# peterdavidfagan/mujoco_robot_environments

Measured on AMD Instinct MI355X. Metric: env steps/sec (whole node), RearrangementEnv batch=4096 at 1/2/4/8 MI355X, higher is better.
Workload: dtype f32

## Files before the change

### mujoco_robot_environments_amd/csrc/mre_dev.h

```cpp
#pragma once
#include <stdint.h>

namespace mre {

constexpr int NB = 20;
constexpr int NRB = 16;
constexpr int GRIP_BODY0 = 8;
constexpr int NV = 39;
constexpr int NRV = 15;
constexpr int NQ = 43;
constexpr int NQP = 44;
constexpr int TRACE_W = 88;
constexpr int TRACE_QVEL = 48;
constexpr int NVP = 40;
constexpr int NU = 8;
constexpr int QFINE = 32;
constexpr int QFINE_ROW = 96;
constexpr int QFINE_CUBE_Q = 32;
constexpr int QFINE_CUBE_V = 60;
static_assert(QFINE_CUBE_Q + 7 * 4 == QFINE_CUBE_V && QFINE_CUBE_V + 6 * 4 <= QFINE_ROW, "qfine row layout");
constexpr int NPROP = 4;
constexpr int NG = 20;
constexpr int PROP_GEOM0 = 12;
constexpr int NPAIR = 128;
// ... 156 lines not shown

struct StepArgs {
  const DevModel* M;
  int N;
  float* qpos;
  float* qvel;
  float* qacc_ws;
  float* qfine;
  float* ctrl;
  const float* ctrl_seq;
  int seq_stride;
  const int* nprops;
  const float* prop_size;
  int nsteps, control_steps, mode;
  unsigned flags;
  const OscConfig* osc;
  int osc_stride;
  const float* osc_target;
  const uint8_t* grip_closed;
  uint8_t* converged;
  float* sites;
  uint32_t* status;
  int* nstep;
  int* stats;
  float* trace;
  int trace_nenv, trace_max, trace_base;
  const uint8_t* env_mask;
  const int* env_order;
  float* geoms;
  float* contacts;
  float* contacts_full;
  int* settle_steps;
  int min_settle_steps;
  const uint8_t* large;
  int want_large;
  float *sv_qpos, *sv_qvel, *sv_qacc_ws, *sv_qfine, *sv_ctrl;
  int* sv_nstep;
  uint32_t* sv_status;
  uint8_t* sv_converged;
  int* launch_info;
  uint8_t* pending;
  int* q_head;
  int* q_tail;
  int* q_buf;
  int* q_acc;
  int* q_done;
  int* q_started;
  const int* q_gen;
  int q_gen_expect;
  int q_wait;
  int* q_err;
  int q_nticks, q_shards, q_cap, q_stride;
  int q_lshards, q_capl;
};
constexpr int QUEUE_TICKS_MAX = 256;
constexpr int QUEUE_SHARDS_MAX = 32;
constexpr int QUEUE_LSHARDS_MAX = 16;

struct SearchArgs {
  const DevModel* M;
  int N;
  float* qpos;
  const int* nprops;
  const float* prop_size;
  const uint8_t* env_mask;
  const long long* env_ids;
  long long env_id_offset;
  unsigned long long seed;
  const int* prop;
  int fixed_prop;
  const double* bounds;
  double shared_bounds[6];
  const int* tick_base;
  long long tick0;
  int max_attempts;
  int yaw_mode;
  double fixed_quat[4];
  float max_dist;
  int commit;
  float* qfine;
  double* pose;
  int* attempts;
  unsigned flags;
};

constexpr int DYN_W = 128;
constexpr int DYN_JAC = 0, DYN_MASS = 42, DYN_BIAS = 91, DYN_POS = 98, DYN_QUAT = 101, DYN_QPOS = 105, DYN_QVEL = 112,
              DYN_PAD = 119;
struct DynArgs {
  const DevModel* M;
  int N;
  const float* qpos;
  const float* qvel;
  const float* qfine;
  const int* nprops;
  const float* prop_size;
  int site;
  float* out;
};

struct SortArgs {
  const DevModel* M;
  int N;
  const float* qpos;
  const int* nprops;
  const double* zones;
// ... 30 lines not shown
```

### mujoco_robot_environments_amd/csrc/mre_env.h

```cpp
#pragma once
#include <hip/hip_runtime.h>

#include <string>
#include <utility>
#include <vector>

#include "../../include/mre.h"
#include "mre_dev.h"
#include "mre_policy.h"

#define HIPCHK(x)                                                                       \
  do {                                                                                  \
    hipError_t e_ = (x);                                                                \
    if (e_ != hipSuccess)                                                               \
      return mre::fail(MRE_ERR_HIP, std::string(#x) + ": " + hipGetErrorString(e_));    \
  } while (0)

struct mre_env {
  int N = 0, device = 0;
  hipStream_t stream = nullptr;
  mre::DevModel* dM = nullptr;
  mre::DevModel hM;
  int solver = MRE_SOLVER_PGS;
  float *qpos = nullptr, *qvel = nullptr, *qacc_ws = nullptr, *ctrl = nullptr;
// ... 29 lines not shown
  std::vector<std::pair<hipEvent_t, hipEvent_t>> events;
  size_t events_used = 0;
  bool fallback = true;
  unsigned base_flags = 0;
  bool large_only = false;
  bool compact_only = false;
  hipStream_t stream2 = nullptr;
  hipEvent_t ev_fork = nullptr, ev_join = nullptr, ev_order = nullptr;
  uint8_t *d_large = nullptr, *mask_r = nullptr;
  float *sv_qpos = nullptr, *sv_qvel = nullptr, *sv_qacc_ws = nullptr, *sv_ctrl = nullptr, *sv_qfine = nullptr;
  uint32_t* sv_status = nullptr;
  uint8_t* sv_converged = nullptr;
  float* contacts = nullptr;
  float* contacts_full = nullptr;
  int* settle_steps = nullptr;
  int* h_launch_info = nullptr;
  int* d_launch_info = nullptr;
  int* h_info_last = nullptr;
  uint8_t* d_pending = nullptr;
  uint8_t* h_large_stage = nullptr;
  uint8_t* d_large_stage = nullptr;
  bool d_large_stale = false;
  std::vector<uint8_t> h_large, h_rerun;
  int n_large = 0;
  long long* d_env_ids = nullptr;
  int *ps_attempts = nullptr, *ps_prop = nullptr, *ps_tick = nullptr, *ps_which = nullptr;
  double *ps_bounds = nullptr, *ps_pose = nullptr, *ps_zones = nullptr, *ps_pick = nullptr;
  int last_settle_max = 0;
  long long n_reruns = 0, n_promotions = 0, n_demotions = 0;
  struct Group {
    int lo = 0, n = 0;
    hipStream_t st = nullptr, st2 = nullptr;
    hipEvent_t ev_fork = nullptr, ev_join = nullptr;
    struct Out {
      mre::StepArgs args;
      hipEvent_t ev_info = nullptr;
      int stage = 0;
    } out[mre::policy::RING];
    int head = 0, nout = 0;
    int cur = 0;
    int* h_order = nullptr;
    int* d_order = nullptr;
  };
  std::vector<Group> groups;
  int* h_grp_order = nullptr;
  int* d_grp_order = nullptr;
  Group qgroup;
  bool queue_ok = true;
  int queue_ticks = 200;
  int queue_waves = 0;
  int queue_shards = 16;
  int queue_lshards = 8;
  bool queue_test_serial = false;
  int queue_spare_large = 8;
  int queue_run_ticks = 100;
  int queue_min_ticks = 32;
  float tick_tail = 0.f;
  bool tick_tail_valid = false;
  float queue_tail_min = 1.45f;
  unsigned tail_samples = 0;
  std::vector<int> tail_scratch;
  int queue_large_waves_max = 0;
  int* h_qlist = nullptr;
  int* q_ws = nullptr;
  int* q_gen = nullptr;
  int* h_q_err = nullptr;
  int* h_qgrp_order = nullptr;
  long n_queue_launches = 0;
  long long n_handovers = 0;
  int queue_last_handovers = 0;
  static constexpr int RING = mre::policy::RING;
  int ring = 2;
  static constexpr int NSTAGE = mre::policy::NSTAGE;
  hipEvent_t ev_main = nullptr;
  float* seq_copy[RING + 1] = {nullptr, nullptr, nullptr, nullptr, nullptr};
  size_t seq_cap = 0;
  unsigned seq_calls = 0;
  double dbg_wait_s = 0, dbg_call_s = 0; long dbg_calls = 0;
  int calls_since_drain = 0, sync_streak = 0;
  bool broken = false;
};

namespace mre {
int fail(int code, const std::string& msg);
int sched_create(mre_env* e);
void sched_destroy(mre_env* e);
int launch_step(mre_env* e, const StepArgs& a, bool settle = false, bool pipeline_ok = true, bool allow_queue = false);
int drain(mre_env* e, bool api_call = false);
}
#define DRAIN(e) do { int rc_ = mre::drain(e, true); if (rc_) return rc_; } while (0)
#define DRAIN_PENDING(e) do { int rc_ = mre::drain(e, false); if (rc_) return rc_; } while (0)

inline int profile_events(mre_env* e, hipEvent_t* e0, hipEvent_t* e1) {
  *e0 = *e1 = nullptr;
  if (!e->profiling) return MRE_OK;
  if (e->events_used == e->events.size()) {
    hipEvent_t x, y;
    HIPCHK(hipEventCreate(&x)); HIPCHK(hipEventCreate(&y));
    e->events.emplace_back(x, y);
  }
  *e0 = e->events[e->events_used].first; *e1 = e->events[e->events_used].second;
  e->events_used++;
  return MRE_OK;
}
```

### mujoco_robot_environments_amd/csrc/mre_kernels.hip

```cpp
#include <hip/hip_runtime.h>

#include "mre_dev.h"
#include "mre_math.h"
#include "mre_collide.h"

namespace mre {
using ModelP = MRE_MODEL_PTR(DevModel);
#if defined(MRE_PHASE_STAMPS) && MRE_PHASE_STAMPS >= 4
__shared__ unsigned long long dbg_acc[4];
#endif

struct OscSm {
  float J[6][7], M[7][7], MiJt[7][6], Li[6][6], Lam[6][6], V[6][6], Jbar[7][6];
  float ep[3], eo[3], F[6], LF[6], tn[7], Jbt[6], xd[6], w[6];
};

struct alignas(8) Blk {
  uint16_t row0;
  uint8_t type, nrows;
  uint8_t rslot;
  uint8_t pa, pb;
  uint8_t primary : 4;
  uint8_t bslot : 4;
};
// ... 1229 lines not shown
    return 1;
  }
}
MRE_DEV bool queue_pop(const StepArgs& a, int l, int home, int& env, int& tick, int& shard) {
  const int S = a.q_shards;
  if (Q_LARGE) {
    const int SL = a.q_lshards;
    for (unsigned idle = 0;; ++idle) {
      int r = 0;
      for (int k = 0; k < SL && r == 0; ++k) {
        const int sh = S + (home + k < SL ? home + k : home + k - SL);
        r = queue_pop_shard(a, l, sh, env, tick);
        if (r != 0) shard = sh;
      }
      if (r != 0) return r > 0;
      if (a.q_wait == 0 || q_load(a.q_done) >= a.N) return false;
      if (idle > 512u && q_load(a.q_started) == 0) return false;
      if (idle > (1u << 18)) return false;
      __builtin_amdgcn_s_sleep(127);
    }
  }
  for (int k = 0; k < S; ++k) {
    const int sh = home + k < S ? home + k : home + k - S;
    const int r = queue_pop_shard(a, l, sh, env, tick);
    if (r != 0) { shard = sh; return r > 0; }
  }
  return false;
}
MRE_DEV void queue_push(const StepArgs& a, int l, int env, int tick, int shard) {
  __builtin_amdgcn_fence(__ATOMIC_RELEASE, "agent");
  asm volatile("s_waitcnt vmcnt(0)" ::: "memory");
  if (l == 0) {
    const int i = __hip_atomic_fetch_add(a.q_tail + shard * QUEUE_TICKS_MAX + tick, 1, __ATOMIC_RELAXED, __HIP_MEMORY_SCOPE_AGENT);
    __hip_atomic_store(q_bucket(a, tick, shard) + i, env + 1, __ATOMIC_RELAXED, __HIP_MEMORY_SCOPE_AGENT);
  }
}

template <bool QUEUE>
MRE_DEV void step_body(const StepArgs& a, Sm& s) {
  OscSm& osc = s.osc;
  const int l = threadIdx.x;
  int env = 0, qtick = 0, qshard = 0;
  if (!QUEUE) {
    if ((int)blockIdx.x >= a.N) return;
    env = a.env_order != nullptr ? a.env_order[blockIdx.x] : (int)blockIdx.x;
  }
  if (QUEUE && !Q_LARGE && l == 0) __hip_atomic_fetch_add(a.q_started, 1, __ATOMIC_RELAXED, __HIP_MEMORY_SCOPE_AGENT);
  if (QUEUE && Q_LARGE && a.q_wait != 0) {
    for (unsigned idle = 0; q_load(a.q_gen) != a.q_gen_expect; ++idle) {
      if (idle > 1024u) return;
      __builtin_amdgcn_s_sleep(127);
    }
  }
 for (;;) {
  if (QUEUE) {
    if (!queue_pop(a, l, (int)(blockIdx.x % (unsigned)(Q_LARGE ? a.q_lshards : a.q_shards)), env, qtick, qshard)) return;
    if (qtick > 0 || Q_LARGE) __builtin_amdgcn_fence(__ATOMIC_ACQUIRE, "agent");
  }
  const int step_lo = QUEUE ? qtick * a.control_steps : 0, step_hi = QUEUE ? step_lo + a.control_steps : a.nsteps;
  if (QUEUE && !Q_LARGE && qtick == 0 && a.large != nullptr && a.large[env] != 0) continue;
  if (!QUEUE || (!Q_LARGE && qtick == 0)) {
#define MRE_PASS_SKIP { if (QUEUE) { if (l == 0) __hip_atomic_fetch_add(a.q_done, 1, __ATOMIC_RELAXED, __HIP_MEMORY_SCOPE_AGENT); continue; } return; }
  if (!QUEUE && a.large != nullptr && (a.large[env] != 0) != (a.want_large != 0)) return;
  if (a.env_mask != nullptr && a.env_mask[env] == 0) {
    if (a.launch_info != nullptr && l < 4) a.launch_info[(size_t)env * 4 + l] = -1;
    MRE_PASS_SKIP;
  }
  if (a.pending != nullptr && a.pending[env] != 0) {
    if (a.launch_info != nullptr && l < 4) a.launch_info[(size_t)env * 4 + l] = l == 0 ? -2 : -1;
    MRE_PASS_SKIP;
  }
#undef MRE_PASS_SKIP
  }
  ModelP M = (ModelP)a.M;

  const bool save = a.sv_qpos != nullptr && step_lo == 0;
  if (l < NQP) {
    const float v = a.qpos[(size_t)env * NQP + l];
    s.qpos[l] = v;
    if (save) a.sv_qpos[(size_t)env * NQP + l] = v;
  }
  if (l < NVP) {
    const float v = a.qvel[(size_t)env * NVP + l], w = a.qacc_ws[(size_t)env * NVP + l];
    s.qvel[l] = v;
    s.qacc[l] = w;
    s.qfrc_con[l] = 0.f;
    if (save) { a.sv_qvel[(size_t)env * NVP + l] = v; a.sv_qacc_ws[(size_t)env * NVP + l] = w; }
  }
  if (l < QFINE) {
    const float v = a.qfine != nullptr ? a.qfine[(size_t)env * QFINE_ROW + l] : 0.f;
    s.qlo[l] = v;
    if (save && a.qfine != nullptr) a.sv_qfine[(size_t)env * QFINE_ROW + l] = v;
  }
  if (save && a.qfine != nullptr && l < QFINE_ROW - QFINE)
    a.sv_qfine[(size_t)env * QFINE_ROW + QFINE + l] = a.qfine[(size_t)env * QFINE_ROW + QFINE + l];
  float cube_lo_keep = 0.f;
  if (QUEUE && !Q_LARGE && a.qfine != nullptr && l < QFINE_ROW - QFINE) cube_lo_keep = a.qfine[(size_t)env * QFINE_ROW + QFINE + l];
  if (l < NU) {
    const float v = a.ctrl[(size_t)env * NU + l];
    s.ctrl[l] = v;
    if (save) a.sv_ctrl[(size_t)env * NU + l] = v;
  }
  if (save && l == 0) {
    if (a.nstep != nullptr) a.sv_nstep[env] = a.nstep[env];
    a.sv_status[env] = a.status[env];
    a.sv_converged[env] = a.converged != nullptr ? a.converged[env] : (uint8_t)0;
  }
  if (l == 0) { s.nprops = a.nprops[env]; s.overflow = 0; s.ncon = 0; s.nefc = 0; s.solver_iters = 0; }
#ifdef MRE_NEWTON
  if (l < 24) s.zrow[l] = 0.f;
#endif
  if (l < NPROP * 3) {
    const float sz = a.prop_size[(size_t)env * NPROP * 3 + l];
    s.prop_size[l / 3][l % 3] = sz;
  }
  MRE_SYNC();
  if (l < NPROP) {
    const float m = M->body_mass[NRB + l];
    const float* z = s.prop_size[l];
    s.prop_mass[l] = m;
    s.prop_inertia[l][0] = m / 3.f * (z[1] * z[1] + z[2] * z[2]);
    s.prop_inertia[l][1] = m / 3.f * (z[0] * z[0] + z[2] * z[2]);
    s.prop_inertia[l][2] = m / 3.f * (z[0] * z[0] + z[1] * z[1]);
  }
  MRE_SYNC();

#if defined(MRE_PHASE_STAMPS) && MRE_PHASE_STAMPS >= 4
  if (l < 4) dbg_acc[l] = 0ull;
#endif
#ifdef MRE_PHASE_STAMPS
  unsigned long long stamp_acc[4] = {0, 0, 0, 0};
  unsigned long long stamp_t = __builtin_amdgcn_s_memtime();
#endif
  bool arm_converged = ((a.flags & F_CONV_CONTINUE) != 0 || (QUEUE && qtick > 0)) && a.converged != nullptr && a.converged[env] != 0;
  float grip_cmd = 0.f;
  const OscConfig* oscp = a.osc + (size_t)env * a.osc_stride;
  int hw_ncon = 0, hw_nefc = 0, hw_nrrow = 0, hw_npp = 0;
  const unsigned long long launch_t0 = __builtin_amdgcn_s_memtime();
  if (a.mode == CTRL_OSC) {
    if (l < 16) s.osc_tgt[l] = a.osc_target[(size_t)env * 16 + l];
    grip_cmd = a.grip_closed[env] ? M->act_ctrlrange[NU - 1][1] : M->act_ctrlrange[NU - 1][0];
    MRE_SYNC();
  }
  int steps_done = 0;
  bool settled = false;
  for (int step = step_lo; step < step_hi; ++step) {
    MRE_STAMP(7);
    position_stage(M, s, l);
    MRE_STAMP(12);
    MRE_STAMP(13);
    gripper_local(M, s, l);
    if ((a.flags & F_NO_CONSTRAINTS) == 0) connect_rows_local(M, s, l);
    MRE_STAMP(14);
    crb_mass_matrix(M, s, l);
    MRE_SYNC();
#ifndef MRE_NEWTON
    factor_robot_regs(s.qM, s.qLD, s.qLDinv);
#endif
    MRE_STAMP(15);
    MRE_STAMP(0);

    velocity_stage(M, s, l);
    MRE_SYNC();
    finger_bias(M, s, l);
    MRE_STAMP(1);
    const bool constrained = (a.flags & F_NO_CONSTRAINTS) == 0;
    if (constrained) {

      collide(M, s, l, false, (a.flags & F_CLIP_ALWAYS) != 0);
      MRE_STAMP(2);
      assemble_constraints(M, s, l);
#ifdef MRE_NEWTON
      nw_build_lists(s, l);
#else
      solve_robot_rows(s, l);
      assemble_blocks(M, s, l);
#endif
      MRE_STAMP(3);
      hw_ncon = max(hw_ncon, s.ncon); hw_nefc = max(hw_nefc, s.nefc);
      hw_nrrow = max(hw_nrrow, s.nrrow); hw_npp = max(hw_npp, s.npp);
    }

    if (a.mode == CTRL_SEQ && (step % a.control_steps) == 0) {
      const int tick = step / a.control_steps;
      if (l < NU) s.ctrl[l] = a.ctrl_seq[((size_t)tick * a.seq_stride + env) * NU + l];
      MRE_SYNC();
    }
    if (a.mode == CTRL_OSC && (step % a.control_steps) == 0) {
      if (step > 0 && osc_converged(M, s, oscp, s.osc_tgt)) arm_converged = true;
      osc_compute(M, s, osc, oscp, s.osc_tgt, l);
      if (l == 0) s.ctrl[NU - 1] = grip_cmd;
      MRE_SYNC();
// ... 88 lines not shown
    MRE_SYNC();
  }
  if (a.nsteps == 0 && (a.flags & F_DETECT) != 0 && a.contacts != nullptr) {
    position_stage(M, s, l);
    collide(M, s, l, (a.flags & F_DETECT_ACTIVE) == 0, (a.flags & F_CLIP_ALWAYS) != 0);
    float* o = a.contacts + (size_t)env * (1 + 3 * CONTACT_EXPORT);
    const int n = s.ncon < CONTACT_EXPORT ? s.ncon : CONTACT_EXPORT;
    if (l == 0) o[0] = s.overflow ? -(float)s.ncon : (float)s.ncon;
    if (l < n) {
      const int pr = s.con_pair[l];
      o[1 + 3 * l] = (float)M->pair_g1[pr]; o[2 + 3 * l] = (float)M->pair_g2[pr]; o[3 + 3 * l] = s.con_dist[l];
      if (a.contacts_full != nullptr) {
        float* f = a.contacts_full + ((size_t)env * CONTACT_EXPORT + l) * 12;
        for (int k = 0; k < 3; k++) f[k] = s.con_pos[l][k];
        for (int k = 0; k < 9; k++) f[3 + k] = s.con_frame[l][k];
      }
    }
    MRE_SYNC();
    if (l == 0) s.overflow = 0;
  }
  const bool q_last = !QUEUE || (qtick + 1 == a.q_nticks && !hand_over);
  if (q_last && (a.mode == CTRL_OSC || a.sites != nullptr || a.geoms != nullptr)) kinematics_only(M, s, l);
  if (a.mode == CTRL_OSC && a.nsteps > 0 && !hand_over) {
    if (q_last && osc_converged(M, s, oscp, s.osc_tgt)) arm_converged = true;
    if (l == 0) {
      if (a.converged != nullptr) a.converged[env] = arm_converged ? 1 : 0;
      if (q_last && !arm_converged && a.status != nullptr && (a.flags & F_CONV_OPEN) == 0) {
        if (QUEUE) __hip_atomic_fetch_or(a.status + env, 1u, __ATOMIC_RELAXED, __HIP_MEMORY_SCOPE_AGENT);
        else a.status[env] |= 1u;
      }
    }
  }
  if (a.geoms != nullptr && l < NG) {
    float p[3], R[9], size[3], rb;
    geom_pose(M, s, l, p, R, size, &rb);
    float* o = a.geoms + ((size_t)env * NG + l) * 16;
    const int pid = M->geom_propid[l];
    const bool active = pid < 0 || pid < s.nprops;
    for (int k = 0; k < 3; k++) o[k] = p[k];
    for (int k = 0; k < 9; k++) o[3 + k] = R[k];
    for (int k = 0; k < 3; k++) o[12 + k] = size[k];
    o[15] = active ? (float)M->geom_type[l] : -1.f;
  }
  if (a.sites != nullptr && q_last) {
    float* o = a.sites + (size_t)env * 16;
    if (l < 3) o[l] = s.site_xpos[M->opt_rec.tcp_site][l];
    if (l >= 3 && l < 6) o[l] = s.site_xpos[M->opt_rec.eef_site][l - 3];
    if (l == 6) {
      float q[4];
      mat2q(q, s.site_xmat[0]);
      o[6] = q[0]; o[7] = q[1]; o[8] = q[2]; o[9] = q[3];
    }
  }
  if (hand_over) {
    if (a.qfine != nullptr && l < QFINE_ROW - QFINE) a.qfine[(size_t)env * QFINE_ROW + QFINE + l] = cube_lo_keep;
  } else {
    if (l < NQP) a.qpos[(size_t)env * NQP + l] = s.qpos[l];
    if (l < NVP) {
      a.qvel[(size_t)env * NVP + l] = s.qvel[l];
      a.qacc_ws[(size_t)env * NVP + l] = l < NV ? s.qacc[l] : 0.f;
    }
    if (l < QFINE && a.qfine != nullptr) a.qfine[(size_t)env * QFINE_ROW + l] = s.qlo[l];
    if (l < NU) a.ctrl[(size_t)env * NU + l] = s.ctrl[l];
  }
  const bool q_more = QUEUE && !hand_over && qtick + 1 < a.q_nticks;
  if (l == 0 && a.launch_info != nullptr) {
    int* li = a.launch_info + (size_t)env * 4;
    unsigned long long dt = (__builtin_amdgcn_s_memtime() - launch_t0) >> 10;
    int moved = 0;
    if (QUEUE) {
      int* qa = a.q_acc + (size_t)env * 4;
      if (qtick > 0 || Q_LARGE) {
        hw_ncon = max(hw_ncon, q_load(qa + 0) & 0xFFFF); hw_nefc = max(hw_nefc, q_load(qa + 1));
        hw_nrrow = max(hw_nrrow, q_load(qa + 2) & 0xFFFF); hw_npp = max(hw_npp, q_load(qa + 2) >> 16);
        dt += (unsigned long long)q_load(qa + 3);
        moved = q_load(qa + 0) >> 16;
      }
      if (hand_over) moved = 1;
      if (q_more || hand_over) { qa[0] = hw_ncon | (moved << 16); qa[1] = hw_nefc; qa[2] = hw_nrrow | (hw_npp << 16); qa[3] = (int)dt; }
      else dt /= (unsigned long long)(qtick + 1);
    }
    if (!q_more && !hand_over) {
#ifdef MRE_LARGE_CAPS
      li[0] = (s.overflow ? 2 : 0) | (moved ? 4 : 0);
#else
      li[0] = s.overflow ? 1 : 0;
#endif
      li[1] = hw_ncon | ((int)(dt < 0x7FFFull ? dt : 0x7FFFull) << 16); li[2] = hw_nefc; li[3] = hw_nrrow | (hw_npp << 16);
    }
  }
#ifndef MRE_LARGE_CAPS
  if (!QUEUE && l == 0 && a.pending != nullptr && s.overflow) a.pending[env] = 1;
#endif
  if (l == 0 && a.status != nullptr && !hand_over) {
    unsigned st = 0;
    for (int k = 0; k < NQ; k++) if (!isfinite(s.qpos[k])) st |= 2u;
    if (s.overflow) st |= 4u;
    if (QUEUE) { if (st) __hip_atomic_fetch_or(a.status + env, st, __ATOMIC_RELAXED, __HIP_MEMORY_SCOPE_AGENT); }
    else a.status[env] |= st;
    if (a.stats != nullptr && a.nsteps > 0) {
      a.stats[env * 4 + 0] = s.ncon; a.stats[env * 4 + 1] = s.nefc;
      a.stats[env * 4 + 2] = s.solver_iters; a.stats[env * 4 + 3] = s.nl;
#ifdef MRE_PHASE_STAMPS
      for (int k = 0; k < 4; k++) a.stats[env * 4 + k] = (int)(stamp_acc[k] >> 4);
#if MRE_PHASE_STAMPS >= 4
      for (int k = 0; k < 4; k++) a.stats[env * 4 + k] = (int)(dbg_acc[k] >> 4);
#endif
#endif
    }
  }
  if (!QUEUE) return;
  if (hand_over) queue_push(a, l, env, qtick, a.q_shards + env % a.q_lshards);
  else if (q_more) queue_push(a, l, env, qtick + 1, qshard);
  else if (l == 0) __hip_atomic_fetch_add(a.q_done, 1, __ATOMIC_RELAXED, __HIP_MEMORY_SCOPE_AGENT);
 }
}

#ifdef MRE_NEWTON
#define MRE_VARIANT(name) name##_newton
#else
#define MRE_VARIANT(name) name
#endif

#ifdef MRE_LARGE_CAPS
__global__ __launch_bounds__(64, 2) void MRE_VARIANT(k_step_large)(StepArgs a) {
  __shared__ Sm s;
  step_body<false>(a, s);
}
}

extern "C" void MRE_VARIANT(mre_launch_step_large)(const mre::StepArgs* args, hipStream_t stream) {
  hipLaunchKernelGGL(mre::MRE_VARIANT(k_step_large), dim3(args->N), dim3(64), 0, stream, *args);
}
namespace mre {
__global__ __launch_bounds__(64, 2) void MRE_VARIANT(k_step_queue_large)(StepArgs a) {
  __shared__ Sm s;
  step_body<true>(a, s);
}
}
extern "C" void MRE_VARIANT(mre_launch_step_queue_large)(const mre::StepArgs* args, int nwaves, hipStream_t stream) {
  hipLaunchKernelGGL(mre::MRE_VARIANT(k_step_queue_large), dim3(nwaves), dim3(64), 0, stream, *args);
}
#else
__global__ __launch_bounds__(64, 2) void MRE_VARIANT(k_step)(StepArgs a) {
  __shared__ Sm s;
  step_body<false>(a, s);
}

__global__ __launch_bounds__(64, 2) void MRE_VARIANT(k_settle)(StepArgs a) {
  __shared__ Sm s;
  step_body<false>(a, s);
}

__global__ __launch_bounds__(64, 2) void MRE_VARIANT(k_step_queue)(StepArgs a) {
  __shared__ Sm s;
  step_body<true>(a, s);
}

#ifdef MRE_NEWTON
}
extern "C" void mre_launch_step_newton(const mre::StepArgs* args, hipStream_t stream) {
  hipLaunchKernelGGL(mre::k_step_newton, dim3(args->N), dim3(64), 0, stream, *args);
}
extern "C" void mre_launch_settle_newton(const mre::StepArgs* args, hipStream_t stream) {
  hipLaunchKernelGGL(mre::k_settle_newton, dim3(args->N), dim3(64), 0, stream, *args);
}
extern "C" void mre_launch_step_queue_newton(const mre::StepArgs* args, int nwaves, hipStream_t stream) {
// ... 346 lines not shown
```

### mujoco_robot_environments_amd/csrc/mre_policy.h

```cpp
#pragma once
#include <algorithm>

#include "mre_dev.h"

namespace mre {
namespace policy {

constexpr int RING = 4;
constexpr int NSTAGE = RING + 1;

inline int info_duration(const int* li) { return li[0] < 0 ? 0 : (li[1] >> 16); }

inline int compact_nrrow_max(bool newton) { return newton ? NRROW_MAX_COMPACT_NEWTON : NRROW_MAX_COMPACT_PGS; }
inline bool near_compact_caps(bool newton, int hw_ncon, int hw_nefc, int hw_nrrow, int hw_npp) {
  return 8 * hw_ncon > 7 * NCON_MAX || 8 * hw_nefc > 7 * NEFC_MAX || 8 * hw_nrrow > 7 * compact_nrrow_max(newton) || 8 * hw_npp > 7 * NPP_MAX;
}
inline bool far_below_compact_caps(bool newton, int hw_ncon, int hw_nefc, int hw_nrrow, int hw_npp) {
  return 8 * hw_ncon <= 5 * NCON_MAX && 8 * hw_nefc <= 5 * NEFC_MAX && 8 * hw_nrrow <= 5 * compact_nrrow_max(newton) && 8 * hw_npp <= 5 * NPP_MAX;
}

enum Action {
  NONE,
  RERUN,
  PROMOTE,
// ... 15 lines not shown
  for (int i = lo; i < lo + n; i++) kmax = std::max(kmax, info_duration(info + 4 * (size_t)i));
  if (kmax == 0) return 0;
  int count[258] = {0};
  auto bucket = [&](int i) { return (int)((long long)info_duration(info + 4 * (size_t)i) * 255 / kmax); };
  for (int i = lo; i < lo + n; i++) count[255 - bucket(i) + 1]++;
  for (int k = 1; k <= 256; k++) count[k] += count[k - 1];
  for (int i = lo; i < lo + n; i++) order[lo + count[255 - bucket(i)]++] = i;
  return kmax;
}

inline bool tick_tail_ratio(const int* info, int lo, int n, int* scratch, float* ratio) {
  size_t m = 0;
  long long sum = 0;
  for (int i = lo; i < lo + n; i++) {
    const int* li = info + 4 * (size_t)i;
    if (li[0] >= 0) { scratch[m++] = li[1] >> 16; sum += li[1] >> 16; }
  }
  if (m < 256 || sum <= 0) return false;
  const size_t k = m - 1 - m / 100;
  std::nth_element(scratch, scratch + k, scratch + m);
  *ratio = (float)scratch[k] * (float)m / (float)sum;
  return true;
}

inline int free_stage(int cur, const int* younger_stages, int nyounger) {
  bool used[NSTAGE] = {false};
  used[cur] = true;
  for (int k = 0; k < nyounger; k++) used[younger_stages[k]] = true;
  int fs = 0;
  while (used[fs]) fs++;
  return fs;
}

inline int queue_large_waves(const int* info_last, const uint8_t* large, int lo, int n, int nl, int last_handovers,
                             int spare_large, int large_waves_max ) {
  int lw = nl + std::max(last_handovers, spare_large);
  double wl = 0, wc = 0;
  for (int i = lo; i < lo + n; i++) {
    const double d = (double)info_duration(info_last + 4 * (size_t)i);
    if (large[i]) wl += d; else wc += d;
  }
  const double ncomp = (double)(n - nl);
  const double r = (wl > 0 && wc > 0) ? wl / wc : (ncomp > 0 ? 1.3 * (double)nl / ncomp : 1e9);
  const double x = r * 160.0 / (26.5 * r + 20.4);
  const int bal = std::max((int)(x * (double)(large_waves_max / 2)), large_waves_max / 4);
  return std::max(std::min(lw, bal), 1);
}

inline bool queue_fits(bool queue_ok, int queue_waves, int N) { return queue_ok && queue_waves > 0 && N > queue_waves; }
inline bool window_wants_queue(int nticks, int queue_min_ticks, bool tick_tail_valid, float tick_tail, float queue_tail_min) {
  return nticks >= queue_min_ticks || (nticks >= 8 && !(tick_tail_valid && tick_tail < queue_tail_min));
}

inline int ring_keep(int nsteps, int ring) { return nsteps <= 50 ? ring - 1 : 0; }

}
}
```

### mujoco_robot_environments_amd/csrc/mre_sched.cpp

```cpp
#include <hip/hip_runtime.h>
#include <chrono>
#include <cstdlib>
#include <cstring>

#include "mre_env.h"
#include "mre_launch.h"

using namespace mre;

static void launch_compact(const mre_env* e, const StepArgs& a, hipStream_t st, bool settle = false) {
  const StepKernels& K = step_kernels(e->solver);
  (settle ? K.settle : K.step)(&a, st);
}
static void launch_large(const mre_env* e, const StepArgs& a, hipStream_t st) { step_kernels(e->solver).large(&a, st); }

static int launch_split(const mre_env* e, const StepArgs& a, bool run_large, bool settle, hipStream_t st, hipStream_t st2,
                        hipEvent_t ev_fork, hipEvent_t ev_join) {
  StepArgs ac = a;
  ac.want_large = 0;
  if (run_large) {
    HIPCHK(hipEventRecord(ev_fork, st));
    HIPCHK(hipStreamWaitEvent(st2, ev_fork, 0));
    StepArgs al = a;
    al.want_large = 1;
// ... 105 lines not shown
  }
  bool any = e->qgroup.nout > 0;
  for (auto& G : e->groups) any = any || G.nout > 0;
  if (!any) return MRE_OK;
  HIPCHK(hipSetDevice(e->device));
  for (auto& G : e->groups) {
    int rc = drain_group(e, G, true);
    if (rc) return rc;
  }
  return drain_group(e, e->qgroup, true);
}

static void guard_args(mre_env* e, StepArgs& a) {
  a.large = e->d_large; a.launch_info = e->d_launch_info;
  a.sv_qpos = e->sv_qpos; a.sv_qvel = e->sv_qvel; a.sv_qacc_ws = e->sv_qacc_ws; a.sv_qfine = e->sv_qfine;
  a.sv_ctrl = e->sv_ctrl; a.sv_status = e->sv_status; a.sv_converged = e->sv_converged; a.sv_nstep = e->sv_nstep;
}

static int launch_group_enqueue(mre_env* e, mre_env::Group& G, const StepArgs& a_full, bool queue) {
  int rc;
  StepArgs a = a_full;
  const size_t N = (size_t)e->N;
  if (G.nout == 0) {
    memcpy(e->h_large_stage + (size_t)G.cur * N + G.lo, e->h_large.data() + G.lo, (size_t)G.n);
    (void)policy::sort_longest_first(e->h_info_last, G.lo, G.n, G.h_order + (size_t)G.cur * N);
  }
  a.N = G.n; a.env_order = G.d_order + (size_t)G.cur * N + G.lo; a.seq_stride = e->N;
  hipEvent_t p0, p1;
  rc = profile_events(e, &p0, &p1);
  if (rc) return rc;
  HIPCHK(hipStreamWaitEvent(G.st, e->ev_main, 0));
  if (p0) HIPCHK(hipEventRecord(p0, G.st));
  guard_args(e, a);
  a.pending = e->d_pending;
  const int slot = (G.head + G.nout) % mre_env::RING;
  a.large = e->d_large_stage + (size_t)G.cur * N;
  a.launch_info = e->d_launch_info + (size_t)slot * 4 * N;
  const uint8_t* const fl = e->h_large_stage + (size_t)G.cur * N;
  if (queue) {
    StepArgs ac = a;
    ac.want_large = 0;
    const StepKernels& K = step_kernels(e->solver);
    const int nt = a.nsteps / a.control_steps, S = e->queue_shards, cap = (G.n + S - 1) / S;
    const int SL = e->queue_lshards, capl = (G.n + SL - 1) / SL;
    constexpr int QS = QUEUE_SHARDS_MAX + QUEUE_LSHARDS_MAX;
    const size_t ctl = 2 * (size_t)QS * QUEUE_TICKS_MAX + 16;
    const size_t stride = (size_t)S * cap + (size_t)SL * capl;
    const size_t words = ctl + 4 * N + (size_t)nt * stride;
    ac.sv_qpos = nullptr;
    ac.q_head = e->q_ws; ac.q_tail = ac.q_head + QS * QUEUE_TICKS_MAX;
    ac.q_done = ac.q_tail + QS * QUEUE_TICKS_MAX; ac.q_started = ac.q_done + 1; ac.q_acc = ac.q_done + 16;
    ac.q_buf = ac.q_acc + 4 * N; ac.q_err = e->h_q_err; ac.q_nticks = nt; ac.q_shards = S; ac.q_cap = cap; ac.q_stride = (int)stride;
    ac.q_lshards = SL; ac.q_capl = capl;
    ac.q_gen = e->q_gen; ac.q_gen_expect = (int)(e->n_queue_launches + 1);
    int* const hl = e->h_qlist + (size_t)(e->n_queue_launches % (mre_env::RING + 1)) * (N + 32);
    int nl = 0;
    for (int j = 0; j < SL; j++) hl[j] = 0;
    memset(hl + 16, 0, (size_t)SL * capl * 4);
    for (int i = G.lo; i < G.lo + G.n; i++)
      if (fl[i]) { const int j = i % SL; hl[16 + (size_t)j * capl + hl[j]++] = i + 1; nl++; }
    StepArgs al = ac;
    al.want_large = 1; al.q_wait = 1;
    const int lw = policy::queue_large_waves(e->h_info_last, fl, G.lo, G.n, nl, e->queue_last_handovers, e->queue_spare_large,
                                             e->queue_large_waves_max);
    hipStream_t const st_large = e->queue_test_serial ? G.st : G.st2;
    K.queue_large(&al, lw, st_large);
    HIPCHK(hipGetLastError());
    HIPCHK(hipEventRecord(G.ev_join, st_large));
    HIPCHK(hipMemsetAsync(e->q_ws, 0, ((words * 4 + 15) / 16) * 16, G.st));
    if (nl > 0) {
      HIPCHK(hipMemcpyAsync(ac.q_buf + (size_t)S * cap, hl + 16, (size_t)SL * capl * 4, hipMemcpyHostToDevice, G.st));
      HIPCHK(hipMemcpy2DAsync(ac.q_tail + S * QUEUE_TICKS_MAX, (size_t)QUEUE_TICKS_MAX * 4, hl, 4, 4, (size_t)SL, hipMemcpyHostToDevice, G.st));
    }
    HIPCHK(hipMemsetD32Async((hipDeviceptr_t)e->q_gen, ac.q_gen_expect, 1, G.st));
    const int nwaves = G.n < e->queue_waves ? G.n : e->queue_waves;
    K.queue(&ac, nwaves, G.st);
    HIPCHK(hipGetLastError());
    al.q_wait = 0;
    const int sweep = G.n < 3 * e->queue_large_waves_max ? G.n : 3 * e->queue_large_waves_max;
    K.queue_large(&al, sweep, G.st);
    e->n_queue_launches++;
    HIPCHK(hipGetLastError());
    HIPCHK(hipStreamWaitEvent(G.st, G.ev_join, 0));
  } else {
    bool run_large = false;
    for (int i = G.lo; i < G.lo + G.n && !run_large; i++) run_large = fl[i] != 0;
    rc = launch_split(e, a, run_large, false, G.st, G.st2, G.ev_fork, G.ev_join);
    if (rc) return rc;
  }
  if (p1) HIPCHK(hipEventRecord(p1, G.st));
  HIPCHK(hipEventRecord(G.out[slot].ev_info, G.st));
  G.out[slot].args = a;
  G.out[slot].stage = G.cur;
  G.nout++;
  return MRE_OK;
}
static int launch_group(mre_env* e, mre_env::Group& G, const StepArgs& a_full, bool queue = false) {
  while (G.nout > policy::ring_keep(a_full.nsteps, e->ring)) {
    int rc = process_oldest(e, G);
    if (rc) return rc;
  }
  int rc = launch_group_enqueue(e, G, a_full, queue);
  if (rc) {
    (void)hipStreamSynchronize(G.st);
    (void)hipStreamSynchronize(G.st2);
    G.nout = 0; G.head = 0;
// ... 80 lines not shown
      e->n_reruns += nrerun;
    }
    if (changed) {
      HIPCHK(hipMemcpyAsync(e->d_large, e->h_large.data(), N, hipMemcpyHostToDevice, e->stream));
      HIPCHK(hipStreamSynchronize(e->stream));
    }
  }
  if (e1) HIPCHK(hipEventRecord(e1, e->stream));
  return MRE_OK;
}

int mre::sched_create(mre_env* e) {
  const int num_envs = e->N;
  const size_t N = (size_t)num_envs;
  int least = 0, greatest = 0;
  HIPCHK(hipDeviceGetStreamPriorityRange(&least, &greatest));
  int ng = 4, min_envs = 512;
  if (const char* g = getenv("MRE_GROUPS")) ng = atoi(g);
  if (const char* g = getenv("MRE_GROUP_MIN")) min_envs = atoi(g);
  if (ng < 1) ng = 1;
  if (ng > 8) ng = 8;
  if (const char* r = getenv("MRE_RING")) { e->ring = atoi(r); if (e->ring < 2) e->ring = 2; if (e->ring > mre_env::RING) e->ring = mre_env::RING; }
  while (ng > 1 && num_envs < min_envs * ng) ng--;
  HIPCHK(hipHostMalloc((void**)&e->h_grp_order, mre_env::NSTAGE * N * 4, hipHostMallocMapped | hipHostMallocCoherent));
  HIPCHK(hipHostGetDevicePointer((void**)&e->d_grp_order, e->h_grp_order, 0));
  for (int k = 0; k < mre_env::NSTAGE; k++)
    for (int i = 0; i < num_envs; i++) e->h_grp_order[(size_t)k * N + i] = i;
  HIPCHK(hipEventCreateWithFlags(&e->ev_main, hipEventDisableTiming));
  e->groups.resize(ng);
  auto& Q = e->qgroup;
  Q.lo = 0; Q.n = num_envs;
  HIPCHK(hipHostMalloc((void**)&e->h_qgrp_order, mre_env::NSTAGE * N * 4, hipHostMallocMapped | hipHostMallocCoherent));
  Q.h_order = e->h_qgrp_order;
  HIPCHK(hipHostGetDevicePointer((void**)&Q.d_order, Q.h_order, 0));
  for (int k = 0; k < mre_env::NSTAGE; k++)
    for (int i = 0; i < num_envs; i++) Q.h_order[(size_t)k * N + i] = i;
  HIPCHK(hipStreamCreateWithPriority(&Q.st, hipStreamNonBlocking, least));
  HIPCHK(hipStreamCreateWithPriority(&Q.st2, hipStreamNonBlocking, greatest));
  HIPCHK(hipEventCreateWithFlags(&Q.ev_fork, hipEventDisableTiming));
  HIPCHK(hipEventCreateWithFlags(&Q.ev_join, hipEventDisableTiming));
  for (auto& o : Q.out) HIPCHK(hipEventCreateWithFlags(&o.ev_info, hipEventDisableTiming));
  if (const char* q = getenv("MRE_QUEUE")) e->queue_ok = atoi(q) != 0;
  if (const char* q = getenv("MRE_QUEUE_TICKS")) { const int v = atoi(q); if (v >= 2 && v <= QUEUE_TICKS_MAX) e->queue_ticks = v; }
  if (e->queue_run_ticks > e->queue_ticks) e->queue_run_ticks = e->queue_ticks;
  hipDeviceProp_t prop;
  HIPCHK(hipGetDeviceProperties(&prop, e->device));
  e->queue_waves = prop.multiProcessorCount * std::min(step_kernels(MRE_SOLVER_PGS).queue_waves_per_cu(),
                                                       step_kernels(MRE_SOLVER_NEWTON).queue_waves_per_cu());
  if (const char* q = getenv("MRE_QUEUE_WAVES")) { const int v = atoi(q); if (v > 0) e->queue_waves = v; }
  if (const char* q = getenv("MRE_QUEUE_SHARDS")) { const int v = atoi(q); if (v >= 1 && v <= QUEUE_SHARDS_MAX) e->queue_shards = v; }
  if (const char* q = getenv("MRE_QUEUE_MIN_TICKS")) { const int v = atoi(q); if (v >= 2) e->queue_min_ticks = v; }
  if (const char* q = getenv("MRE_QUEUE_TAIL_MIN")) { const float v = (float)atof(q); if (v > 0.f) e->queue_tail_min = v; }
  if (const char* q = getenv("MRE_QUEUE_TEST_SERIAL")) e->queue_test_serial = atoi(q) != 0;
  if (const char* q = getenv("MRE_QUEUE_SPARE_LARGE")) { const int v = atoi(q); if (v >= 0) e->queue_spare_large = v; }
  e->queue_large_waves_max = 2 * prop.multiProcessorCount;
  if (const char* q = getenv("MRE_QUEUE_LSHARDS")) { const int v = atoi(q); if (v >= 1 && v <= QUEUE_LSHARDS_MAX) e->queue_lshards = v; }
  HIPCHK(hipMalloc(&e->q_ws, ((2 * (size_t)(QUEUE_SHARDS_MAX + QUEUE_LSHARDS_MAX) * QUEUE_TICKS_MAX + 16 + 4 * N +
                               (size_t)QUEUE_TICKS_MAX * (2 * N + QUEUE_SHARDS_MAX + QUEUE_LSHARDS_MAX)) * 4 + 15) / 16 * 16));
  HIPCHK(hipMalloc(&e->q_gen, 64));
  HIPCHK(hipMemsetAsync(e->q_gen, 0, 64, e->stream));
  HIPCHK(hipHostMalloc((void**)&e->h_qlist, (size_t)(mre_env::RING + 1) * (N + 32) * 4, hipHostMallocDefault));
  HIPCHK(hipHostMalloc((void**)&e->h_q_err, 64, hipHostMallocMapped | hipHostMallocCoherent));
  *e->h_q_err = 0;
  for (int g = 0; g < ng; g++) {
    auto& G = e->groups[g];
    G.h_order = e->h_grp_order; G.d_order = e->d_grp_order;
    G.lo = (int)((long long)num_envs * g / ng);
    G.n = (int)((long long)num_envs * (g + 1) / ng) - G.lo;
    int pr = 0;
    const char* gp = getenv("MRE_GROUP_PRIORITY");
    if (!(gp && atoi(gp) == 0)) { pr = greatest + g; if (pr > least) pr = least; }
    if (const char* map = getenv("MRE_GROUP_PRIO_MAP")) {
      if ((int)strlen(map) > g && map[g] >= '0' && map[g] <= '9') { pr = greatest + (map[g] - '0'); if (pr > least) pr = least; }
    }
    HIPCHK(hipStreamCreateWithPriority(&G.st, hipStreamNonBlocking, pr));
    HIPCHK(hipStreamCreateWithPriority(&G.st2, hipStreamNonBlocking, pr));
    HIPCHK(hipEventCreateWithFlags(&G.ev_fork, hipEventDisableTiming));
    HIPCHK(hipEventCreateWithFlags(&G.ev_join, hipEventDisableTiming));
    for (auto& o : G.out) HIPCHK(hipEventCreateWithFlags(&o.ev_info, hipEventDisableTiming));
  }
  return MRE_OK;
}

void mre::sched_destroy(mre_env* e) {
  auto free_group = [](mre_env::Group& G) {
    if (G.st) { (void)hipStreamSynchronize(G.st); (void)hipStreamDestroy(G.st); }
    if (G.st2) { (void)hipStreamSynchronize(G.st2); (void)hipStreamDestroy(G.st2); }
    if (G.ev_fork) (void)hipEventDestroy(G.ev_fork);
    if (G.ev_join) (void)hipEventDestroy(G.ev_join);
    for (auto& O : G.out) if (O.ev_info) (void)hipEventDestroy(O.ev_info);
  };
  for (auto& G : e->groups) free_group(G);
  free_group(e->qgroup);
  if (e->q_ws) (void)hipFree(e->q_ws);
  if (e->q_gen) (void)hipFree(e->q_gen);
  if (e->h_q_err) (void)hipHostFree(e->h_q_err);
  if (e->h_qlist) (void)hipHostFree(e->h_qlist);
  if (e->h_qgrp_order) (void)hipHostFree(e->h_qgrp_order);
  if (e->ev_main) (void)hipEventDestroy(e->ev_main);
  if (e->h_grp_order) (void)hipHostFree(e->h_grp_order);
}
```

Measured before the change: 24.78 million.

## Keep env resident across consecutive queue ticks to skip pop/push and state reload

In the persistent queue kernel, a workgroup that finishes a tick now keeps the same environment for the next tick within a run of q_run ticks. It skips the queue push/pop, the global state reload into shared memory, and the launch_info writeback in between. Only per-step scratch such as contact counts and constraint forces is reset. Runs default to 2 ticks when there are enough ticks, which cuts queue atomics and global traffic but reduces load-balancing granularity. It also adds optional phase-timing instrumentation.

```diff
diff --git a/mujoco_robot_environments_amd/csrc/mre_dev.h b/mujoco_robot_environments_amd/csrc/mre_dev.h
--- a/mujoco_robot_environments_amd/csrc/mre_dev.h
+++ b/mujoco_robot_environments_amd/csrc/mre_dev.h
@@ -232,6 +232,7 @@
   int* q_err;
   int q_nticks, q_shards, q_cap, q_stride;
   int q_lshards, q_capl;
+  int q_run;
 };
 constexpr int QUEUE_TICKS_MAX = 256;
 constexpr int QUEUE_SHARDS_MAX = 32;
diff --git a/mujoco_robot_environments_amd/csrc/mre_env.h b/mujoco_robot_environments_amd/csrc/mre_env.h
--- a/mujoco_robot_environments_amd/csrc/mre_env.h
+++ b/mujoco_robot_environments_amd/csrc/mre_env.h
@@ -105,6 +105,7 @@
   int queue_shards = 16;
   int queue_lshards = 8;
   bool queue_test_serial = false;
+  int queue_run = 0;
   int queue_spare_large = 8;
   int queue_run_ticks = 100;
   int queue_min_ticks = 32;
diff --git a/mujoco_robot_environments_amd/csrc/mre_kernels.hip b/mujoco_robot_environments_amd/csrc/mre_kernels.hip
--- a/mujoco_robot_environments_amd/csrc/mre_kernels.hip
+++ b/mujoco_robot_environments_amd/csrc/mre_kernels.hip
@@ -1305,10 +1305,34 @@
       __builtin_amdgcn_s_sleep(127);
     }
   }
+  bool q_keep = false;
+  int q_tick0 = 0;
+  bool arm_converged = false;
+  float grip_cmd = 0.f, cube_lo_keep = 0.f;
+  int hw_ncon = 0, hw_nefc = 0, hw_nrrow = 0, hw_npp = 0;
+  unsigned long long q_dt = 0;
+#if defined(MRE_PHASE_STAMPS) && MRE_PHASE_STAMPS == 9
+  unsigned long long q_seg[4] = {0, 0, 0, 0};
+  unsigned long long q_seg_t = 0;
+#endif
  for (;;) {
-  if (QUEUE) {
+  if (QUEUE && !q_keep) {
+#if defined(MRE_PHASE_STAMPS) && MRE_PHASE_STAMPS == 9
+    q_seg_t = __builtin_amdgcn_s_memtime();
+    const bool q_got = queue_pop(a, l, (int)(blockIdx.x % (unsigned)(Q_LARGE ? a.q_lshards : a.q_shards)), env, qtick, qshard);
+    { const unsigned long long now_ = __builtin_amdgcn_s_memtime(); q_seg[0] += now_ - q_seg_t; q_seg_t = now_; }
+    if (!q_got) {
+      if (!Q_LARGE && l == 0 && a.stats != nullptr) {
+        for (int k = 0; k < 3; k++) a.stats[blockIdx.x * 4 + k] = (int)(q_seg[k] >> 4);
+        a.stats[blockIdx.x * 4 + 3] = (int)q_seg[3];
+      }
+      return;
+    }
+#else
     if (!queue_pop(a, l, (int)(blockIdx.x % (unsigned)(Q_LARGE ? a.q_lshards : a.q_shards)), env, qtick, qshard)) return;
+#endif
     if (qtick > 0 || Q_LARGE) __builtin_amdgcn_fence(__ATOMIC_ACQUIRE, "agent");
+    q_tick0 = qtick; hw_ncon = 0; hw_nefc = 0; hw_nrrow = 0; hw_npp = 0; q_dt = 0;
   }
   const int step_lo = QUEUE ? qtick * a.control_steps : 0, step_hi = QUEUE ? step_lo + a.control_steps : a.nsteps;
   if (QUEUE && !Q_LARGE && qtick == 0 && a.large != nullptr && a.large[env] != 0) continue;
@@ -1327,6 +1351,7 @@
   }
   ModelP M = (ModelP)a.M;
 
+  if (!q_keep) {
   const bool save = a.sv_qpos != nullptr && step_lo == 0;
   if (l < NQP) {
     const float v = a.qpos[(size_t)env * NQP + l];
@@ -1347,7 +1372,6 @@
   }
   if (save && a.qfine != nullptr && l < QFINE_ROW - QFINE)
     a.sv_qfine[(size_t)env * QFINE_ROW + QFINE + l] = a.qfine[(size_t)env * QFINE_ROW + QFINE + l];
-  float cube_lo_keep = 0.f;
   if (QUEUE && !Q_LARGE && a.qfine != nullptr && l < QFINE_ROW - QFINE) cube_lo_keep = a.qfine[(size_t)env * QFINE_ROW + QFINE + l];
   if (l < NU) {
     const float v = a.ctrl[(size_t)env * NU + l];
@@ -1377,6 +1401,13 @@
     s.prop_inertia[l][2] = m / 3.f * (z[0] * z[0] + z[1] * z[1]);
   }
   MRE_SYNC();
+  } else {
+    if (l < NVP) { s.qfrc_con[l] = 0.f; if (l >= NV) s.qacc[l] = 0.f; }
+    if (l == 0) { s.overflow = 0; s.ncon = 0; s.nefc = 0; s.solver_iters = 0; }
+    if (!Q_LARGE && a.qfine != nullptr && l < QFINE_ROW - QFINE) cube_lo_keep = a.qfine[(size_t)env * QFINE_ROW + QFINE + l];
+    if (a.converged == nullptr) arm_converged = false;
+    MRE_SYNC();
+  }
 
 #if defined(MRE_PHASE_STAMPS) && MRE_PHASE_STAMPS >= 4
   if (l < 4) dbg_acc[l] = 0ull;
@@ -1385,12 +1416,13 @@
   unsigned long long stamp_acc[4] = {0, 0, 0, 0};
   unsigned long long stamp_t = __builtin_amdgcn_s_memtime();
 #endif
-  bool arm_converged = ((a.flags & F_CONV_CONTINUE) != 0 || (QUEUE && qtick > 0)) && a.converged != nullptr && a.converged[env] != 0;
-  float grip_cmd = 0.f;
+  if (!q_keep) arm_converged = ((a.flags & F_CONV_CONTINUE) != 0 || (QUEUE && qtick > 0)) && a.converged != nullptr && a.converged[env] != 0;
   const OscConfig* oscp = a.osc + (size_t)env * a.osc_stride;
-  int hw_ncon = 0, hw_nefc = 0, hw_nrrow = 0, hw_npp = 0;
   const unsigned long long launch_t0 = __builtin_amdgcn_s_memtime();
-  if (a.mode == CTRL_OSC) {
+#if defined(MRE_PHASE_STAMPS) && MRE_PHASE_STAMPS == 9
+  if (QUEUE && !q_keep) { q_seg[1] += launch_t0 - q_seg_t; q_seg[3] += 1; }
+#endif
+  if (a.mode == CTRL_OSC && !q_keep) {
     if (l < 16) s.osc_tgt[l] = a.osc_target[(size_t)env * 16 + l];
     grip_cmd = a.grip_closed[env] ? M->act_ctrlrange[NU - 1][1] : M->act_ctrlrange[NU - 1][0];
     MRE_SYNC();
@@ -1585,6 +1617,11 @@
       o[6] = q[0]; o[7] = q[1]; o[8] = q[2]; o[9] = q[3];
     }
   }
+  const bool q_more = QUEUE && !hand_over && qtick + 1 < a.q_nticks;
+  const bool q_keep_next = q_more && qtick + 1 < min((qtick / a.q_run + 1) * a.q_run, a.q_nticks);
+#if defined(MRE_PHASE_STAMPS) && MRE_PHASE_STAMPS == 9
+  if (QUEUE && !q_keep_next) q_seg_t = __builtin_amdgcn_s_memtime();
+#endif
   if (hand_over) {
     if (a.qfine != nullptr && l < QFINE_ROW - QFINE) a.qfine[(size_t)env * QFINE_ROW + QFINE + l] = cube_lo_keep;
   } else {
@@ -1596,14 +1633,15 @@
     if (l < QFINE && a.qfine != nullptr) a.qfine[(size_t)env * QFINE_ROW + l] = s.qlo[l];
     if (l < NU) a.ctrl[(size_t)env * NU + l] = s.ctrl[l];
   }
-  const bool q_more = QUEUE && !hand_over && qtick + 1 < a.q_nticks;
-  if (l == 0 && a.launch_info != nullptr) {
+  if (a.launch_info != nullptr) {
+    unsigned long long dt = (__builtin_amdgcn_s_memtime() - launch_t0) >> 10;
+    if (QUEUE) { q_dt += dt; dt = q_dt; }
+    if (l == 0 && !q_keep_next) {
     int* li = a.launch_info + (size_t)env * 4;
-    unsigned long long dt = (__builtin_amdgcn_s_memtime() - launch_t0) >> 10;
     int moved = 0;
     if (QUEUE) {
       int* qa = a.q_acc + (size_t)env * 4;
-      if (qtick > 0 || Q_LARGE) {
+      if (q_tick0 > 0 || Q_LARGE) {
         hw_ncon = max(hw_ncon, q_load(qa + 0) & 0xFFFF); hw_nefc = max(hw_nefc, q_load(qa + 1));
         hw_nrrow = max(hw_nrrow, q_load(qa + 2) & 0xFFFF); hw_npp = max(hw_npp, q_load(qa + 2) >> 16);
         dt += (unsigned long long)q_load(qa + 3);
@@ -1621,6 +1659,7 @@
 #endif
       li[1] = hw_ncon | ((int)(dt < 0x7FFFull ? dt : 0x7FFFull) << 16); li[2] = hw_nefc; li[3] = hw_nrrow | (hw_npp << 16);
     }
+    }
   }
 #ifndef MRE_LARGE_CAPS
   if (!QUEUE && l == 0 && a.pending != nullptr && s.overflow) a.pending[env] = 1;
@@ -1631,6 +1670,9 @@
     if (s.overflow) st |= 4u;
     if (QUEUE) { if (st) __hip_atomic_fetch_or(a.status + env, st, __ATOMIC_RELAXED, __HIP_MEMORY_SCOPE_AGENT); }
     else a.status[env] |= st;
+#if defined(MRE_PHASE_STAMPS) && MRE_PHASE_STAMPS == 9
+    if (!QUEUE)
+#endif
     if (a.stats != nullptr && a.nsteps > 0) {
       a.stats[env * 4 + 0] = s.ncon; a.stats[env * 4 + 1] = s.nefc;
       a.stats[env * 4 + 2] = s.solver_iters; a.stats[env * 4 + 3] = s.nl;
@@ -1643,9 +1685,14 @@
     }
   }
   if (!QUEUE) return;
+  q_keep = q_keep_next;
+  if (q_keep) { ++qtick; continue; }
   if (hand_over) queue_push(a, l, env, qtick, a.q_shards + env % a.q_lshards);
   else if (q_more) queue_push(a, l, env, qtick + 1, qshard);
   else if (l == 0) __hip_atomic_fetch_add(a.q_done, 1, __ATOMIC_RELAXED, __HIP_MEMORY_SCOPE_AGENT);
+#if defined(MRE_PHASE_STAMPS) && MRE_PHASE_STAMPS == 9
+  q_seg[2] += __builtin_amdgcn_s_memtime() - q_seg_t;
+#endif
  }
 }
 
diff --git a/mujoco_robot_environments_amd/csrc/mre_policy.h b/mujoco_robot_environments_amd/csrc/mre_policy.h
--- a/mujoco_robot_environments_amd/csrc/mre_policy.h
+++ b/mujoco_robot_environments_amd/csrc/mre_policy.h
@@ -91,6 +91,11 @@
   return nticks >= queue_min_ticks || (nticks >= 8 && !(tick_tail_valid && tick_tail < queue_tail_min));
 }
 
+inline int queue_next_boundary(int t, int run, int nticks) { return std::min((t / run + 1) * run, nticks); }
+constexpr int QUEUE_RUN_DEFAULT = 2;
+constexpr int QUEUE_RUN_MIN_ITEMS = 8;
+inline int queue_default_run(int nticks) { return nticks >= QUEUE_RUN_MIN_ITEMS * QUEUE_RUN_DEFAULT ? QUEUE_RUN_DEFAULT : 1; }
+
 inline int ring_keep(int nsteps, int ring) { return nsteps <= 50 ? ring - 1 : 0; }
 
 }
diff --git a/mujoco_robot_environments_amd/csrc/mre_sched.cpp b/mujoco_robot_environments_amd/csrc/mre_sched.cpp
--- a/mujoco_robot_environments_amd/csrc/mre_sched.cpp
+++ b/mujoco_robot_environments_amd/csrc/mre_sched.cpp
@@ -181,6 +181,7 @@
     ac.q_done = ac.q_tail + QS * QUEUE_TICKS_MAX; ac.q_started = ac.q_done + 1; ac.q_acc = ac.q_done + 16;
     ac.q_buf = ac.q_acc + 4 * N; ac.q_err = e->h_q_err; ac.q_nticks = nt; ac.q_shards = S; ac.q_cap = cap; ac.q_stride = (int)stride;
     ac.q_lshards = SL; ac.q_capl = capl;
+    ac.q_run = e->queue_run > 0 ? e->queue_run : policy::queue_default_run(nt);
     ac.q_gen = e->q_gen; ac.q_gen_expect = (int)(e->n_queue_launches + 1);
     int* const hl = e->h_qlist + (size_t)(e->n_queue_launches % (mre_env::RING + 1)) * (N + 32);
     int nl = 0;
@@ -367,6 +368,7 @@
   if (const char* q = getenv("MRE_QUEUE_MIN_TICKS")) { const int v = atoi(q); if (v >= 2) e->queue_min_ticks = v; }
   if (const char* q = getenv("MRE_QUEUE_TAIL_MIN")) { const float v = (float)atof(q); if (v > 0.f) e->queue_tail_min = v; }
   if (const char* q = getenv("MRE_QUEUE_TEST_SERIAL")) e->queue_test_serial = atoi(q) != 0;
+  if (const char* q = getenv("MRE_QUEUE_RUN")) { const int v = atoi(q); if (v >= 1 && v <= QUEUE_TICKS_MAX) e->queue_run = v; }
   if (const char* q = getenv("MRE_QUEUE_SPARE_LARGE")) { const int v = atoi(q); if (v >= 0) e->queue_spare_large = v; }
   e->queue_large_waves_max = 2 * prop.multiProcessorCount;
   if (const char* q = getenv("MRE_QUEUE_LSHARDS")) { const int v = atoi(q); if (v >= 1 && v <= QUEUE_LSHARDS_MAX) e->queue_lshards = v; }
```

Measured after the change: 25.13 million (median of 6 runs). Within noise of the previous version (+1.4%).
